# ivanalberico/End-To-End-Self-Supervised-SLAM

Hardware: AMD Instinct MI355X
Metric: online refinement steps/sec @640x480, seq_len=60 (higher is better)
Workload: dtype f32

## Files before the change

### end-to-end-self-supervised-slam_amd/csrc/conv.hip

```cpp
#include <cassert>
#include <type_traits>

#include "e2e_common.h"

typedef float f4v __attribute__((ext_vector_type(4)));
typedef float f16v __attribute__((ext_vector_type(16)));

#define CBK 16

enum { ACT_NONE = 0, ACT_RELU = 1, ACT_ELU = 2, ACT_DISP = 3 };

struct ConvArgs {
    const float* src0;
    const float* src1;
    const float* w;
    const float* scale;
    const float* shift;
    const float* res;
    float* out;
    int B, Hs, Ws;
    int Cin, C1, up;
    int Hd, Wd;
    int Ncols, ldw;
    int KH, KW, stride, pad, pad_mode;
// ... 764 lines not shown
#pragma unroll
            for (int kk = 0; kk < CB / 2; ++kk) {
                av[kk] = As[buf][kk * 2 + khalf][arow_l];
                bv[kk] = Bs[buf][kk * 2 + khalf][wn * 32 + (lane & 31)];
            }
#pragma unroll
            for (int kk = 0; kk < CB / 2; ++kk) acc = __builtin_amdgcn_mfma_f32_32x32x2f32(av[kk], bv[kk], acc, 0, 0, 0);
            __builtin_amdgcn_sched_group_barrier(0x100, CB / 2, 0);
            __builtin_amdgcn_sched_group_barrier(0x008, CB / 2, 0);
            __builtin_amdgcn_sched_barrier(0);
            store_chunk(buf ^ 1, buf ^ 1);
            __syncthreads();
        };
        {
            int c = cb;
            for (; c + 1 < ce; c += 2) {
                chunk_step(c, std::integral_constant<int, 0>{});
                chunk_step(c + 1, std::integral_constant<int, 1>{});
            }
            if (c < ce) chunk_step(c, std::integral_constant<int, 0>{});
        }
        const unsigned sl_off = (unsigned)((wave * 4 * 64 + lane) * 16);
        if (cb != 0) {
            const __amdgpu_buffer_rsrc_t rsl = __builtin_amdgcn_make_buffer_rsrc((void*)(s.slabs + (int64_t)g * (BM * BN)), 0, BM * BN * 4, 0x00020000);
            float v[16];
#pragma unroll
            for (int r = 0; r < 16; ++r) {
                v[r] = acc[r];
                asm volatile("" : "+v"(v[r]));
            }
#pragma unroll
            for (int q = 0; q < 4; ++q) {
                const f4v t = {v[4 * q], v[4 * q + 1], v[4 * q + 2], v[4 * q + 3]};
                __builtin_amdgcn_raw_buffer_store_b128(__builtin_bit_cast(__attribute__((__vector_size__(4 * sizeof(unsigned)))) unsigned, t), rsl, sl_off + q * 64 * 16, 0, SK_SC1);
            }
            asm volatile("s_waitcnt vmcnt(0)" ::: "memory");
            __syncthreads();
            if (tid == 0) __hip_atomic_store(&s.flags[g], 1u, __ATOMIC_RELAXED, __HIP_MEMORY_SCOPE_AGENT);
        } else {
            if (ce != s.C) {
                const int64_t tile_end = (int64_t)(tile + 1) * s.C;
                int h_last = g;
                for (int h = g + 1; h < s.G && s.I * h / s.G < tile_end; ++h) h_last = h;
                if (tid == 0) {
                    for (int h = g + 1; h <= h_last; ++h) {
                        unsigned spins = 0;
                        while (__hip_atomic_load(&s.flags[h], __ATOMIC_RELAXED, __HIP_MEMORY_SCOPE_AGENT) == 0u) {
                            __builtin_amdgcn_s_sleep(2);
                            if (++spins > (1u << 24)) { __hip_atomic_store(&s.flags[SK_ERR_INDEX], 1u, __ATOMIC_RELAXED, __HIP_MEMORY_SCOPE_AGENT); break; }
                        }
                    }
                    __builtin_amdgcn_fence(__ATOMIC_ACQUIRE, "agent");
                }
                asm volatile("s_waitcnt vmcnt(0)" ::: "memory");
                __syncthreads();
                for (int h = g + 1; h <= h_last; ++h) {
                    const __amdgpu_buffer_rsrc_t rsl = __builtin_amdgcn_make_buffer_rsrc((void*)(s.slabs + (int64_t)h * (BM * BN)), 0, BM * BN * 4, 0x00020000);
                    f4v t[4];
#pragma unroll
                    for (int q = 0; q < 4; ++q) t[q] = __builtin_bit_cast(f4v, __builtin_amdgcn_raw_buffer_load_b128(rsl, sl_off + q * 64 * 16, 0, SK_SC1));
#pragma unroll
                    for (int q = 0; q < 4; ++q)
#pragma unroll
                        for (int e = 0; e < 4; ++e) acc[4 * q + e] += t[q][e];
                }
                if (tid == 0)
                    for (int h = g + 1; h <= h_last; ++h) __hip_atomic_store(&s.flags[h], 0u, __ATOMIC_RELAXED, __HIP_MEMORY_SCOPE_AGENT);
            }
            const EpiRsrc er = make_epi_rsrc<TRANSPOSED>(a);
            epilogue_block<TRANSPOSED>(a, er, acc, c0 + wn * 32 + (lane & 31), n0 + wm * 32 + 4 * khalf, Ntot);
        }
        it += ce - cb;
    }
}

struct ThinArgs {
    const float* src;
    const float* w;
    const float* bias;
    float* out;
    int B, Hsrc, Wsrc, Hd, Wd, ldw, act, org, flip;
};

template <int CIN, int UP, bool REFLECT, int TH>
__global__ __launch_bounds__(256) void k_conv3x3_thin(ThinArgs a) {
    constexpr int TW = 64, PH = TH + 2, PW = TW + 2, PWS = 72, PLANE = PH * PWS, KQ = CIN / 4;
    static_assert(PLANE % 32 == 16, "the two channel planes a half-wave reads must sit 16 banks apart");
    __shared__ float patch[CIN * PLANE];
    const int tid = threadIdx.x, lane = tid & 63, wave = tid >> 6, l16 = lane & 15, kq = lane >> 4;
    const int x0 = blockIdx.x * TW, y0 = blockIdx.y * TH, b = blockIdx.z;
    const int HD = a.Hsrc * UP, WD = a.Wsrc * UP;
    float wreg[9][KQ];
#pragma unroll
    for (int t = 0; t < 9; ++t)
#pragma unroll
        for (int j = 0; j < KQ; ++j) wreg[t][j] = a.w[(int64_t)((a.flip ? 8 - t : t) * CIN + 4 * j + kq) * a.ldw + l16];
    const float* sb = a.src + (int64_t)b * a.Hsrc * a.Wsrc * CIN;
    for (int idx = tid; idx < PH * PW * KQ; idx += 256) {
        const int q = (UP == 2) ? idx / (PH * PW) : idx % KQ, pix = (UP == 2) ? idx % (PH * PW) : idx / KQ;
        const int py = pix / PW, px = pix - py * PW;
        int Y = y0 - a.org + py, X = x0 - a.org + px;
        bool ok = true;
        if (REFLECT) {
            Y = min(max(reflect1(Y, HD), 0), HD - 1);
            X = min(max(reflect1(X, WD), 0), WD - 1);
        } else {
            ok = Y >= 0 && Y < HD && X >= 0 && X < WD;
        }
        f4v v = {0.f, 0.f, 0.f, 0.f};
        if (ok) v = *(const f4v*)(sb + ((int64_t)(Y / UP) * a.Wsrc + (X / UP)) * CIN + q * 4);
#pragma unroll
        for (int e = 0; e < 4; ++e) patch[(q * 4 + e) * PLANE + py * PWS + px] = v[e];
    }
    __syncthreads();
    const float bv = a.bias ? a.bias[l16] : 0.f;
    float* ob = a.out + (int64_t)b * a.Hd * a.Wd * 16;
#pragma unroll 1
    for (int g2 = 0; g2 < TH; g2 += 2) {
        const int g0 = wave * TH + g2, g1 = g0 + 1;
        const int r0 = g0 >> 2, c0 = (g0 & 3) * 16, r1 = g1 >> 2, c1 = (g1 & 3) * 16;
        f4v acc0 = {0.f, 0.f, 0.f, 0.f}, acc1 = {0.f, 0.f, 0.f, 0.f};
        const float* p0 = patch + kq * PLANE + r0 * PWS + c0 + l16;
        const float* p1 = patch + kq * PLANE + r1 * PWS + c1 + l16;
#pragma unroll
        for (int t = 0; t < 9; ++t) {
            const int off = (t / 3) * PWS + (t % 3);
#pragma unroll
            for (int j = 0; j < KQ; ++j) {
                acc0 = __builtin_amdgcn_mfma_f32_16x16x4f32(p0[4 * j * PLANE + off], wreg[t][j], acc0, 0, 0, 0);
                acc1 = __builtin_amdgcn_mfma_f32_16x16x4f32(p1[4 * j * PLANE + off], wreg[t][j], acc1, 0, 0, 0);
            }
        }
#pragma unroll
        for (int h = 0; h < 2; ++h) {
            const f4v acc = h ? acc1 : acc0;
            const int y = y0 + (h ? r1 : r0), xb = x0 + (h ? c1 : c0) + 4 * kq;
            if (y >= a.Hd) continue;
#pragma unroll
            for (int i = 0; i < 4; ++i)
                if (xb + i < a.Wd) ob[((int64_t)y * a.Wd + xb + i) * 16 + l16] = apply_act(acc[i] + bv, a.act);
        }
    }
}

struct StemArgs {
    const float* src;
    const float* w;
    const float* scale;
    const float* shift;
    float* out;
    int B, Hs, Ws, Hd, Wd, ldw, act;
    float in_sub, in_mul;
};

__global__ __launch_bounds__(256) void k_conv7x7_stem(StemArgs a) {
    constexpr int TH = 4, TW = 32, PH = 2 * TH + 6, PW = 2 * TW + 5, ROW = 208, NJ = 37;
    __shared__ float patch[PH * ROW];
    const int tid = threadIdx.x, lane = tid & 63, wave = tid >> 6, l16 = lane & 15, kq = lane >> 4;
    const int x0 = blockIdx.x * TW, y0 = blockIdx.y * TH, b = blockIdx.z;
    const int co = 16 * wave + l16;
    float wreg[NJ];
    int offk[NJ];
#pragma unroll
    for (int j = 0; j < NJ; ++j) {
        const int k = 4 * j + kq;
        wreg[j] = k < 147 ? a.w[(int64_t)k * a.ldw + co] : 0.f;
        offk[j] = k + (k / 21) * (ROW - 21);
    }
    const float* sb = a.src + (int64_t)b * a.Hs * a.Ws * 3;
    for (int idx = tid; idx < PH * ROW; idx += 256) {
        const int py = idx / ROW, e = idx - py * ROW;
        const int Y = 2 * y0 - 3 + py, X = 2 * x0 - 3 + e / 3;
        const bool ok = e < 3 * PW && Y >= 0 && Y < a.Hs && X >= 0 && X < a.Ws;
        patch[idx] = ok ? (sb[((int64_t)Y * a.Ws + X) * 3 + (e - (e / 3) * 3)] - a.in_sub) * a.in_mul : 0.f;
    }
    __syncthreads();
    const float sc = a.scale ? a.scale[co] : 1.f, sh = a.shift ? a.shift[co] : 0.f;
    float* ob = a.out + (int64_t)b * a.Hd * a.Wd * 64;
#pragma unroll 1
    for (int g = 0; g < 2 * TH; g += 2) {
        const int r = g >> 1;
        const float* p0 = patch + 2 * r * ROW + 6 * l16;
        const float* p1 = p0 + 6 * 16;
        f4v acc0 = {0.f, 0.f, 0.f, 0.f}, acc1 = {0.f, 0.f, 0.f, 0.f};
#pragma unroll
        for (int j = 0; j < NJ; ++j) {
            acc0 = __builtin_amdgcn_mfma_f32_16x16x4f32(p0[offk[j]], wreg[j], acc0, 0, 0, 0);
            acc1 = __builtin_amdgcn_mfma_f32_16x16x4f32(p1[offk[j]], wreg[j], acc1, 0, 0, 0);
        }
        const int y = y0 + r;
        if (y >= a.Hd) continue;
#pragma unroll
        for (int h = 0; h < 2; ++h) {
            const f4v acc = h ? acc1 : acc0;
            const int xb = x0 + 16 * h + 4 * kq;
#pragma unroll
            for (int i = 0; i < 4; ++i)
                if (xb + i < a.Wd) ob[((int64_t)y * a.Wd + xb + i) * 64 + co] = apply_act(fmaf(acc[i], sc, sh), a.act);
        }
    }
}

__global__ __launch_bounds__(256) void k_conv_splitk_epilogue(const float* __restrict__ slab, int S, int64_t total, int Ncols,
                                                              const float* __restrict__ scale, const float* __restrict__ shift,
                                                              const float* res, float* out, int act, const float* __restrict__ xin, int dact,
                                                              const float* __restrict__ pre) {
    for (int64_t i = (int64_t)blockIdx.x * 256 + threadIdx.x; i < total; i += (int64_t)gridDim.x * 256) {
        float v = 0.f;
        for (int z = 0; z < S; ++z) v += slab[(int64_t)z * total + i];
        const int col = (int)(i % Ncols);
        v = fmaf(v, scale ? scale[col] : 1.f, shift ? shift[col] : 0.f);
        if (pre) v += pre[i];
        if (dact) v *= act_deriv(xin[i], dact);
        if (res) v += res[i];
        out[i] = apply_act(v, act);
    }
}

__global__ __launch_bounds__(256) void k_conv_splitk_epilogue_cls(const float* __restrict__ slab, int64_t cls_rows, int B, int Hd, int Wd, int Ncols,
                                                                  int KH, int KW, int off, const float* res, float* out, const float* __restrict__ xin,
                                                                  int dact, const float* __restrict__ pre) {
    const unsigned colq = (unsigned)Ncols >> 2, totalq = (unsigned)B * Hd * Wd * colq;
    for (unsigned q = blockIdx.x * 256u + threadIdx.x; q < totalq; q += gridDim.x * 256u) {
        unsigned t = q;
        const unsigned cq = t % colq; t /= colq;
        const unsigned x = t % Wd; t /= Wd;
        const unsigned y = t % Hd;
        const unsigned b = t / Hd;
        const int py = y & 1, px = x & 1;
        const int kh0 = (py + off) & 1, kw0 = (px + off) & 1;
        const int ntap = ((KH - kh0 + 1) / 2) * ((KW - kw0 + 1) / 2);
        const int Hc = (Hd - py + 1) / 2, Wc = (Wd - px + 1) / 2;
        const int64_t row = ((int64_t)b * Hc + (y >> 1)) * Wc + (x >> 1);
        f4v v = {0.f, 0.f, 0.f, 0.f};
        for (int z = 0; z < ntap; ++z) v += *(const f4v*)(slab + (((int64_t)z * 4 + (py * 2 + px)) * cls_rows + row) * Ncols + cq * 4);
        if (pre) v += ((const f4v*)pre)[q];
        if (dact) {
            const f4v xv = ((const f4v*)xin)[q];
#pragma unroll
            for (int k = 0; k < 4; ++k) v[k] *= act_deriv(xv[k], dact);
        }
        if (res) v += ((const f4v*)res)[q];
        ((f4v*)out)[q] = v;
    }
}

__global__ __launch_bounds__(256) void k_conv_splitk_epilogue4(const float* __restrict__ slab, int S, unsigned totalq, int Ncols,
                                                               const float* __restrict__ scale, const float* __restrict__ shift,
                                                               const float* res, float* out, int act, const float* __restrict__ xin, int dact,
                                                               const float* __restrict__ pre) {
    const unsigned colq = (unsigned)Ncols >> 2;
    for (unsigned q = blockIdx.x * 256u + threadIdx.x; q < totalq; q += gridDim.x * 256u) {
        f4v v = {0.f, 0.f, 0.f, 0.f};
        for (int z = 0; z < S; ++z) v += ((const f4v*)slab)[(int64_t)z * totalq + q];
        const int col = (int)(q % colq) * 4;
        const f4v sc = scale ? *(const f4v*)(scale + col) : (f4v){1.f, 1.f, 1.f, 1.f};
        const f4v sh = shift ? *(const f4v*)(shift + col) : (f4v){0.f, 0.f, 0.f, 0.f};
#pragma unroll
        for (int k = 0; k < 4; ++k) v[k] = fmaf(v[k], sc[k], sh[k]);
        if (pre) v += ((const f4v*)pre)[q];
        if (dact) {
            const f4v xv = ((const f4v*)xin)[q];
#pragma unroll
            for (int k = 0; k < 4; ++k) v[k] *= act_deriv(xv[k], dact);
        }
        if (res) v += ((const f4v*)res)[q];
#pragma unroll
        for (int k = 0; k < 4; ++k) v[k] = apply_act(v[k], act);
        ((f4v*)out)[q] = v;
    }
}

struct WgradArgs {
    const float* dz;
    const float* src0;
    const float* src1;
    float* slabs;
    int B, Hs, Ws, Cin, C1, up;
    int Ho, Wo, Cout;
    int KH, KW, stride, pad, pad_mode;
    int Ngemm;
// ... 1655 lines not shown
        if (workspace && cls_wgs < 500 && a.KH == 3 && a.KW == 3 && a.Cin % cb == 0 && a.Ncols % 4 == 0 && total < (1ll << 31) && !a.scale && !a.shift &&
            a.act == ACT_NONE) {
            a.ksplit = CLS_TAP_SLICES; a.cps = a.Cin / cb; a.cls_rows = Nc;
            p.g = dim3((unsigned)(4 * ((Nc + c.bm - 1) / c.bm)), (unsigned)((a.Ncols + c.bn - 1) / c.bn), (unsigned)CLS_TAP_SLICES);
            p.tail = GT_CLS;
            return p;
        }
        p.g = dim3((unsigned)(4 * ((Nc + c.bm - 1) / c.bm)), (unsigned)((a.Ncols + c.bn - 1) / c.bn));
        return p;
    }
    const GemmCfg c = choose_cfg(Ntot, a.Ncols, K, cb, workspace != nullptr, force);
    p.c = c;
    if (c.S < 0 && workspace && vec == 4 && K % cb == 0 && a.Cin % cb == 0) {
        p.kind = GK_STREAMK;
        p.G = -c.S;
        return p;
    }
    if (c.S > 1) {
        const int nchunks = (K + cb - 1) / cb;
        a.cps = (nchunks + c.S - 1) / c.S;
        const int Sz = (nchunks + a.cps - 1) / a.cps;
        a.ksplit = Sz;
        if (Sz > 1) {
            p.g = dim3((unsigned)((Ntot + c.bm - 1) / c.bm), (unsigned)((a.Ncols + c.bn - 1) / c.bn), (unsigned)Sz);
            const int64_t total = Ntot * a.Ncols;
            p.tail = (a.Ncols % 4 == 0 && total < (1ll << 31)) ? GT_SPLITK4 : GT_SPLITK;
            return p;
        }
        a.ksplit = 1; a.cps = 0;
    }
    p.g = dim3((unsigned)((Ntot + c.bm - 1) / c.bm), (unsigned)((a.Ncols + c.bn - 1) / c.bn));
    return p;
}

template <bool TR>
static void launch_gemm_main(ConvArgs& a, const GemmLaunch& p, float* workspace_all, hipStream_t st) {
    if (p.kind == GK_SCALAR) hipLaunchKernelGGL((k_conv_gemm<4, 1, 1, 2, 1, TR, 16>), p.g, dim3(256), 0, st, a);
    else if (p.kind == GK_STREAMK) launch_streamk<TR>(a, p.cb, p.G, workspace_all, st);
    else launch_tile<TR>(a, p.cb, p.c, p.g, st);
}

static void launch_gemm_tail(const ConvArgs& a, const GemmLaunch& p, hipStream_t st) {
    const int64_t total = (int64_t)a.B * a.Hd * a.Wd * a.Ncols;
    if (p.tail == GT_CLS)
        hipLaunchKernelGGL(k_conv_splitk_epilogue_cls, dim3(egrid(total / 4)), dim3(256), 0, st, a.slab, a.cls_rows, a.B, a.Hd, a.Wd, a.Ncols, a.KH, a.KW, a.off,
                           a.res, a.out, a.xin, a.dact, a.pre);
    else if (p.tail == GT_SPLITK4)
        hipLaunchKernelGGL(k_conv_splitk_epilogue4, dim3(egrid(total / 4)), dim3(256), 0, st, a.slab, a.ksplit, (unsigned)(total / 4), a.Ncols, a.scale, a.shift,
                           a.res, a.out, a.act, a.xin, a.dact, a.pre);
    else if (p.tail == GT_SPLITK)
        hipLaunchKernelGGL(k_conv_splitk_epilogue, dim3(egrid(total)), dim3(256), 0, st, a.slab, a.ksplit, total, a.Ncols, a.scale, a.shift, a.res, a.out, a.act,
                           a.xin, a.dact, a.pre);
}

template <bool TR>
static void launch_gemm(ConvArgs a, int vec, float* workspace_all, GemmCfg force, hipStream_t st) {
    const GemmLaunch p = plan_gemm<TR>(a, vec, workspace_all, force);
    launch_gemm_main<TR>(a, p, workspace_all, st);
    launch_gemm_tail(a, p, st);
}

extern "C" {

int e2e_conv_weight_layouts(const float* w, int Cout, int Cin, int KH, int KW, float* w_fwd, int ld_fwd, float* w_bwd,
                            int ld_bwd, void* stream) {
    E2E_REQUIRE(w && Cout > 0 && Cin > 0 && KH > 0 && KW > 0 && (w_fwd || w_bwd), E2E_ERR_ARG, "e2e_conv_weight_layouts: bad argument");
    E2E_REQUIRE((!w_fwd || (ld_fwd >= Cout && ld_fwd % 4 == 0)) && (!w_bwd || (ld_bwd >= Cin && ld_bwd % 4 == 0)), E2E_ERR_ARG,
                "e2e_conv_weight_layouts: leading dimensions must cover the columns and be multiples of 4");
    hipLaunchKernelGGL(k_weight_layouts, dim3(egrid((int64_t)Cout * Cin * KH * KW)), dim3(256), 0, (hipStream_t)stream, w, Cout, Cin, KH,
                       KW, w_fwd, ld_fwd, w_bwd, ld_bwd);
    E2E_LAUNCH_CHECK("e2e_conv_weight_layouts");
    return E2E_OK;
}

static int device_cus() {
    static const int cus = [] {
        int dev = 0, n = 0;
        if (hipGetDevice(&dev) != hipSuccess || hipDeviceGetAttribute(&n, hipDeviceAttributeMultiprocessorCount, dev) != hipSuccess || n <= 0) n = 256;
        return n;
    }();
    return cus;
}

int e2e_conv_weight_layouts_batched(const long long* desc, int nlayers, void* stream) {
    E2E_REQUIRE(desc && nlayers > 0, E2E_ERR_ARG, "e2e_conv_weight_layouts_batched: bad argument");
    const int grid = device_cus() * 8;
    for (int l0 = 0; l0 < nlayers; l0 += WL_MAXL)
        hipLaunchKernelGGL(k_weight_layouts_batched, dim3(grid), dim3(256), 0, (hipStream_t)stream, desc + (int64_t)l0 * 10, nlayers - l0 < WL_MAXL ? nlayers - l0 : WL_MAXL);
    E2E_LAUNCH_CHECK("e2e_conv_weight_layouts_batched");
    return E2E_OK;
}

int64_t e2e_conv2d_splitk_workspace_floats(int64_t rows, int cols, int K) {
    if (K % 16 != 0) return 0;
    int smax = 1;
    bool sk = false;
    for (int cb = 16; cb <= 32; cb += 16) {
        const GemmCfg c = choose_cfg(rows, cols, K, cb, true);
        if (c.S > smax) smax = c.S;
        if (c.S < 0) sk = true;
    }
    int64_t n = smax > 1 ? (int64_t)smax * rows * cols : 0;
    if (sk && n < (int64_t)SK_MAX_G * 64 * 64) n = (int64_t)SK_MAX_G * 64 * 64;
    return n ? n + SK_FLAG_FLOATS : 0;
}

int64_t e2e_conv2d_bwd_data_workspace_floats(int B, int Hd, int Wd, int cols, int K, int stride) {
    const int64_t plain = e2e_conv2d_splitk_workspace_floats((int64_t)B * Hd * Wd, cols, K);
    if (stride != 2) return plain;
    const int64_t cls = SK_FLAG_FLOATS + cls_slab_floats(B, Hd, Wd, cols);
    return cls > plain ? cls : plain;
}

int64_t e2e_conv_tuned_workspace_floats(int64_t rows, int cols) {
    int64_t n = (int64_t)16 * rows * cols;
    if (n < (int64_t)SK_MAX_G * 64 * 64) n = (int64_t)SK_MAX_G * 64 * 64;
    return n + SK_FLAG_FLOATS;
}
int e2e_conv_workspace_flag_floats(void) { return SK_FLAG_FLOATS; }
int e2e_conv_streamk_error_index(void) { return SK_ERR_INDEX; }

int e2e_conv_gemm_choice(int64_t rows, int cols, int K, int chunk_depth, int allow_split, int* out3) {
    E2E_REQUIRE(out3 && rows > 0 && cols > 0 && K > 0 && (chunk_depth == 16 || chunk_depth == 32), E2E_ERR_ARG, "e2e_conv_gemm_choice: bad argument");
    const GemmCfg c = choose_cfg(rows, cols, K, chunk_depth, allow_split != 0);
    out3[0] = c.bm; out3[1] = c.bn; out3[2] = c.S;
    return E2E_OK;
}

struct ConvGeom { int B, Hs, Ws, Cin, Cout, Ho, Wo, KH, KW, stride, pad, pad_mode, C1, up; float in_sub, in_mul; };
#define GEOM_LAYER(g) ConvGeom g{}; g.B = B; g.Hs = Hs; g.Ws = Ws; g.Cin = Cin; g.Cout = Cout; g.KH = KH; g.KW = KW; g.stride = stride; g.pad = pad; g.pad_mode = pad_mode
#define GEOM_SOURCES(g) g.C1 = C1; g.up = up; g.in_sub = in_sub; g.in_mul = in_mul
#define GEOM_OUTPUT(g) g.Ho = Ho; g.Wo = Wo
#define GEOM_BWD_DATA(g) GEOM_LAYER(g); GEOM_OUTPUT(g)
#define GEOM_BWD_WEIGHT(g) GEOM_LAYER(g); GEOM_OUTPUT(g); GEOM_SOURCES(g)
#define GEOM_WGRAD_QUERY(g) ConvGeom g{}; g.B = B; g.Ho = Ho; g.Wo = Wo; g.Cin = Cin; g.Cout = Cout; g.KH = KH; g.KW = KW
struct FwdOps { const float *src0, *src1, *w_fwd; int ld_fwd; const float *scale, *shift, *residual; float* out; int act; };
struct BwdDataOps { const float* dz; const float* w_bwd; int ld_bwd; float* dxp; int accumulate; const float* x_in; int in_act; const float* pre_add; };
struct WgradIn { const float *dz, *src0, *src1; float* workspace; };

static int fwd_setup(const FwdOps& f, const ConvGeom& g, ConvArgs& a_out, int& vec_out, const char* who) {
    const int B = g.B, Hs = g.Hs, Ws = g.Ws, Cin = g.Cin, Cout = g.Cout, KH = g.KH, KW = g.KW, stride = g.stride, pad = g.pad, pad_mode = g.pad_mode;
    const int C1 = g.C1, up = g.up, ld_fwd = f.ld_fwd;
    E2E_REQUIRE(f.src0 && f.w_fwd && f.out && B > 0 && Hs > 0 && Ws > 0 && Cin > 0 && Cout > 0 && KH > 0 && KW > 0, E2E_ERR_ARG, "%s: bad argument", who);
    E2E_REQUIRE(up == 1 || up == 2, E2E_ERR_ARG, "%s: upsample factor must be 1 or 2", who);
    E2E_REQUIRE(C1 > 0 && C1 <= Cin && (C1 == Cin || f.src1), E2E_ERR_ARG, "%s: bad channel split", who);
    E2E_REQUIRE(pad_mode == 0 || (pad_mode == 1 && pad == 1 && Hs >= 2 && Ws >= 2), E2E_ERR_ARG, "%s: reflection padding needs pad == 1", who);
    E2E_REQUIRE(stride == 1 || stride == 2, E2E_ERR_ARG, "%s: stride must be 1 or 2", who);
    E2E_REQUIRE(Hs % up == 0 && Ws % up == 0 && ld_fwd % 4 == 0 && ld_fwd >= Cout, E2E_ERR_ARG, "%s: bad sizes", who);
    E2E_REQUIRE(pad >= 0 && Hs + 2 * pad >= KH && Ws + 2 * pad >= KW, E2E_ERR_ARG, "%s: the kernel must fit the padded input (pad >= 0)", who);
    const int vec = (Cin % 16 == 0 && (C1 == Cin || C1 % 16 == 0)) ? 4 : 1;
    E2E_REQUIRE(vec == 4 || (C1 == Cin && up == 1), E2E_ERR_ARG, "%s: the scalar path (Cin %% 16 != 0) takes a single full-resolution source", who);
    E2E_REQUIRE((int64_t)B * Hs * Ws * Cin * 4 < (1ll << 30) && (int64_t)KH * KW * Cin * ld_fwd * 4 < (1ll << 31), E2E_ERR_ARG,
                "%s: activations must stay below 1 GB, weights below 2 GB (32-bit buffer offsets with out-of-range markers)", who);
    E2E_REQUIRE(vec != 4 || (KH <= 3 && KW <= 3), E2E_ERR_ARG, "%s: the channel-quad loader takes kernels up to 3 x 3", who);
    ConvArgs a{};
    a.src0 = f.src0; a.src1 = f.src1; a.w = f.w_fwd; a.scale = f.scale; a.shift = f.shift; a.res = f.residual; a.out = f.out;
    a.B = B; a.Hs = Hs; a.Ws = Ws; a.Cin = Cin; a.C1 = C1; a.up = up;
    a.Hd = (Hs + 2 * pad - KH) / stride + 1; a.Wd = (Ws + 2 * pad - KW) / stride + 1;
    a.Ncols = Cout; a.ldw = ld_fwd; a.KH = KH; a.KW = KW; a.stride = stride; a.pad = pad; a.pad_mode = pad_mode; a.off = 0; a.act = f.act;
    a.in_sub = g.in_sub; a.in_mul = g.in_mul;
    a_out = a; vec_out = vec;
    return E2E_OK;
}

static int conv_fwd_impl(const FwdOps& f, const ConvGeom& g, float* workspace, GemmCfg force, void* stream) {
    const int B = g.B, Hs = g.Hs, Ws = g.Ws, Cin = g.Cin, Cout = g.Cout, KH = g.KH, KW = g.KW, stride = g.stride, pad = g.pad, pad_mode = g.pad_mode;
    const int C1 = g.C1, up = g.up, ld_fwd = f.ld_fwd;
    ConvArgs a;
    int vec;
    const int rc = fwd_setup(f, g, a, vec, "e2e_conv2d_fwd");
    if (rc != E2E_OK) return rc;
    if (!force.bm && KH == 7 && KW == 7 && stride == 2 && pad == 3 && pad_mode == 0 && Cin == 3 && Cout == 64 && C1 == Cin && up == 1 && !f.residual && ld_fwd >= 64) {
        StemArgs t{f.src0, f.w_fwd, f.scale, f.shift, f.out, B, Hs, Ws, a.Hd, a.Wd, ld_fwd, f.act, g.in_sub, g.in_mul};
        hipLaunchKernelGGL(k_conv7x7_stem, dim3((a.Wd + 31) / 32, (a.Hd + 3) / 4, B), dim3(256), 0, (hipStream_t)stream, t);
    }
    else if (!force.bm && KH == 3 && KW == 3 && stride == 1 && pad == 1 && pad_mode == 1 && Cout == 16 && C1 == Cin && !f.scale && !f.residual && ld_fwd >= 16 &&
        ((Cin == 16 && up == 2) || (Cin == 32 && up == 1))) {
        ThinArgs t{f.src0, f.w_fwd, f.shift, f.out, B, Hs / up, Ws / up, Hs, Ws, ld_fwd, f.act, 1, 0};
        if (Cin == 16) hipLaunchKernelGGL((k_conv3x3_thin<16, 2, true, 8>), dim3((Ws + 63) / 64, (Hs + 7) / 8, B), dim3(256), 0, (hipStream_t)stream, t);
        else hipLaunchKernelGGL((k_conv3x3_thin<32, 1, true, 4>), dim3((Ws + 63) / 64, (Hs + 3) / 4, B), dim3(256), 0, (hipStream_t)stream, t);
    } else
        launch_gemm<false>(a, vec, workspace, force, (hipStream_t)stream);
    E2E_LAUNCH_CHECK("e2e_conv2d_fwd");
    return E2E_OK;
}

int e2e_conv2d_fwd(const float* src0, const float* src1, int C1, int up, const float* w_fwd, int ld_fwd, const float* scale,
                   const float* shift, const float* residual, float* out, int B, int Hs, int Ws, int Cin, int Cout, int KH,
                   int KW, int stride, int pad, int pad_mode, int act, float in_sub, float in_mul, float* workspace, void* stream) {
    GEOM_LAYER(g); GEOM_SOURCES(g);
    return conv_fwd_impl(FwdOps{src0, src1, w_fwd, ld_fwd, scale, shift, residual, out, act}, g, workspace, GemmCfg{0, 0, 0}, stream);
}

static bool tuning_ok(int tile_m, int tile_n, int ksplit) {
    if (tile_m == 0) return true;
    if (ksplit < 0) return tile_m == 64 && tile_n == 64 && -ksplit <= SK_MAX_G;
    return tile_max_cb(tile_m, tile_n) != 0 && ksplit >= 1 && ksplit <= 16;
}

int e2e_conv2d_fwd_tuned(const float* src0, const float* src1, int C1, int up, const float* w_fwd, int ld_fwd, const float* scale,
                         const float* shift, const float* residual, float* out, int B, int Hs, int Ws, int Cin, int Cout, int KH,
                         int KW, int stride, int pad, int pad_mode, int act, float in_sub, float in_mul, float* workspace, int tile_m, int tile_n,
                         int ksplit, void* stream) {
    E2E_REQUIRE(tuning_ok(tile_m, tile_n, ksplit), E2E_ERR_ARG, "e2e_conv2d_fwd_tuned: unsupported decomposition %d x %d / %d", tile_m, tile_n, ksplit);
    GEOM_LAYER(g); GEOM_SOURCES(g);
    return conv_fwd_impl(FwdOps{src0, src1, w_fwd, ld_fwd, scale, shift, residual, out, act}, g, workspace, GemmCfg{tile_m, tile_n, ksplit}, stream);
}

struct EntryOps {
    const float* x;
    const float *w1_fwd; int ld1; const float *scale1, *shift1; float* out1; int act1; float* workspace1;
    const float* wd_fwd; int ldd; const float *gamma, *beta, *mean, *var; float eps; float *bn_scale, *bn_shift, *bn_rstd, *z, *y;
};
struct EntryPlan { ConvArgs a1, ad; int vec1, vecd; GemmLaunch p1, pd; ConvGeom g1, gd; bool paired; };

static int fwd_entry_plan(const EntryOps& q, const ConvGeom& g, EntryPlan& P, const char* who) {
    E2E_REQUIRE(q.gamma && q.beta && q.mean && q.var && q.bn_scale && q.bn_shift && q.bn_rstd && q.z && q.y, E2E_ERR_ARG, "%s: bad argument", who);
    E2E_REQUIRE(g.pad_mode == 0 && g.C1 == g.Cin && g.up == 1, E2E_ERR_ARG, "%s: a stage entry reads one zero-padded full-resolution source", who);
    P.g1 = g;
    P.gd = g; P.gd.KH = P.gd.KW = 1; P.gd.pad = 0;
    int rc = fwd_setup(FwdOps{q.x, nullptr, q.w1_fwd, q.ld1, q.scale1, q.shift1, nullptr, q.out1, q.act1}, P.g1, P.a1, P.vec1, who);
    if (rc != E2E_OK) return rc;
    rc = fwd_setup(FwdOps{q.x, nullptr, q.wd_fwd, q.ldd, nullptr, nullptr, nullptr, q.z, ACT_NONE}, P.gd, P.ad, P.vecd, who);
    if (rc != E2E_OK) return rc;
    E2E_REQUIRE(P.a1.Hd == P.ad.Hd && P.a1.Wd == P.ad.Wd, E2E_ERR_ARG, "%s: the two branches must produce the same output grid", who);
    P.paired = false;
    if (P.vec1 != 4 || P.vecd != 4 || g.Cout < 128) return E2E_OK;
    P.p1 = plan_gemm<false>(P.a1, 4, q.workspace1, GemmCfg{0, 0, 0});
    P.pd = plan_gemm<false>(P.ad, 4, nullptr, GemmCfg{0, 0, 0});
    auto t14 = [](const GemmLaunch& p) { return p.kind == GK_TILE && p.cb == 32 && p.c.bm == 32 && p.c.bn == 128; };
    P.paired = t14(P.p1) && t14(P.pd) && P.pd.tail == GT_NONE && P.ad.ksplit == 1 && P.pd.g.z == 1;
    return E2E_OK;
}

int e2e_conv2d_fwd_entry_pair(const float* x, const float* w1_fwd, int ld1, const float* scale1, const float* shift1, float* out1, int act1,
                              float* workspace1, const float* wd_fwd, int ldd, const float* gamma, const float* beta, const float* running_mean,
                              const float* running_var, float eps, float* bn_scale, float* bn_shift, float* bn_rstd, float* z, float* y, int B, int Hs,
                              int Ws, int Cin, int Cout, int KH, int KW, int stride, int pad, void* stream) {
    const int pad_mode = 0, C1 = Cin, up = 1;
    const float in_sub = 0.f, in_mul = 1.f;
    GEOM_LAYER(g); GEOM_SOURCES(g);
    const EntryOps q{x, w1_fwd, ld1, scale1, shift1, out1, act1, workspace1, wd_fwd, ldd, gamma, beta, running_mean, running_var, eps, bn_scale, bn_shift, bn_rstd, z, y};
    EntryPlan P;
    int rc = fwd_entry_plan(q, g, P, "e2e_conv2d_fwd_entry_pair");
    if (rc != E2E_OK) return rc;
    const hipStream_t st = (hipStream_t)stream;
    if (!P.paired) {
        rc = conv_fwd_impl(FwdOps{x, nullptr, w1_fwd, ld1, scale1, shift1, nullptr, out1, act1}, P.g1, workspace1, GemmCfg{0, 0, 0}, stream);
        if (rc != E2E_OK) return rc;
        rc = conv_fwd_impl(FwdOps{x, nullptr, wd_fwd, ldd, nullptr, nullptr, nullptr, z, ACT_NONE}, P.gd, nullptr, GemmCfg{0, 0, 0}, stream);
        if (rc != E2E_OK) return rc;
        rc = e2e_bn_fold(gamma, beta, running_mean, running_var, eps, bn_scale, bn_shift, bn_rstd, Cout, stream);
        if (rc != E2E_OK) return rc;
        return e2e_affine_fwd(z, bn_scale, bn_shift, nullptr, 0, y, (int64_t)B * P.ad.Hd * P.ad.Wd * Cout, Cout, stream);
    }
    FwdPairGrid pg;
    pg.agx = P.p1.g.x; pg.agy = P.p1.g.y; pg.agz = P.p1.g.z;
    pg.bgx = P.pd.g.x; pg.bgy = P.pd.g.y;
    pg.first = (pg.agx * pg.agy * pg.agz + 7u) / 8u * 8u;
    const BnFoldArgs bn{gamma, beta, running_mean, running_var, eps, bn_scale, bn_shift, bn_rstd, y};
    hipLaunchKernelGGL(k_conv_fwd_pair, dim3(pg.first + pg.bgx * pg.bgy), dim3(256), 0, st, P.a1, P.ad, bn, pg);
    launch_gemm_tail(P.a1, P.p1, st);
    E2E_LAUNCH_CHECK("e2e_conv2d_fwd_entry_pair");
    return E2E_OK;
}

int e2e_conv2d_fwd_entry_pair_is_one_launch(int ld1, int ldd, int has_workspace1, int B, int Hs, int Ws, int Cin, int Cout, int KH, int KW, int stride, int pad) {
    static float nowhere[4];
    float* const p = nowhere;
    const int pad_mode = 0, C1 = Cin, up = 1;
    const float in_sub = 0.f, in_mul = 1.f;
    GEOM_LAYER(g); GEOM_SOURCES(g);
    const EntryOps q{p, p, ld1, p, p, p, ACT_RELU, has_workspace1 ? p : nullptr, p, ldd, p, p, p, p, 0.f, p, p, p, p, p};
    EntryPlan P;
    if (fwd_entry_plan(q, g, P, "e2e_conv2d_fwd_entry_pair_is_one_launch") != E2E_OK) return 0;
    return P.paired ? 1 : 0;
}

static int bwd_data_setup(const BwdDataOps& d, const ConvGeom& g, GemmCfg force, hipStream_t stream, ConvArgs& a, bool& done, bool dry = false) {
    const int B = g.B, Hs = g.Hs, Ws = g.Ws, Cin = g.Cin, Cout = g.Cout, Ho = g.Ho, Wo = g.Wo, KH = g.KH, KW = g.KW, stride = g.stride, pad = g.pad;
    const int pad_mode = g.pad_mode, ld_bwd = d.ld_bwd;
    done = false;
    E2E_REQUIRE(d.pre_add == nullptr || pad_mode == 0, E2E_ERR_ARG, "e2e_conv2d_bwd_data: the pre-activation addend takes a zero-padded layer");
    E2E_REQUIRE(d.in_act == 0 || (d.x_in && (d.in_act == ACT_RELU || d.in_act == ACT_ELU) && pad_mode == 0), E2E_ERR_ARG,
                "e2e_conv2d_bwd_data: the fused input-activation derivative takes ReLU / ELU, the activation's output and a zero-padded layer");
    E2E_REQUIRE(d.dz && d.w_bwd && d.dxp && B > 0 && Cin > 0 && Cout > 0 && Cout % 16 == 0, E2E_ERR_ARG, "e2e_conv2d_bwd_data: bad argument (Cout %% 16 == 0)");
    E2E_REQUIRE(ld_bwd % 4 == 0 && ld_bwd >= Cin && (stride == 1 || stride == 2), E2E_ERR_ARG, "e2e_conv2d_bwd_data: bad sizes");
    E2E_REQUIRE((int64_t)B * Ho * Wo * Cout * 4 < (1ll << 30) && (int64_t)KH * KW * Cout * ld_bwd * 4 < (1ll << 31) && KH <= 3 && KW <= 3, E2E_ERR_ARG,
                "e2e_conv2d_bwd_data: gradients must stay below 1 GB, weights below 2 GB (32-bit buffer offsets), kernels up to 3 x 3");
    if (!force.bm && KH == 3 && KW == 3 && stride == 1 && pad == 1 && pad_mode == 1 && Cin == 16 && Cout == 16 && !d.accumulate && !d.in_act && !d.pre_add && ld_bwd >= 16) {
        ThinArgs t{d.dz, d.w_bwd, nullptr, d.dxp, B, Ho, Wo, Hs + 2, Ws + 2, ld_bwd, ACT_NONE, 2, 1};
        if (!dry) hipLaunchKernelGGL((k_conv3x3_thin<16, 1, false, 8>), dim3((Ws + 2 + 63) / 64, (Hs + 2 + 7) / 8, B), dim3(256), 0, stream, t);
        done = true;
        return E2E_OK;
    }
    a = ConvArgs{};
    a.src0 = d.dz; a.src1 = nullptr; a.w = d.w_bwd; a.out = d.dxp;
    a.B = B; a.Hs = Ho; a.Ws = Wo; a.Cin = Cout; a.C1 = Cout; a.up = 1;
    const int pp = pad_mode == 1 ? pad : 0;
    a.Hd = Hs + 2 * pp; a.Wd = Ws + 2 * pp; a.off = pad_mode == 1 ? 0 : pad;
    a.Ncols = Cin; a.ldw = ld_bwd; a.KH = KH; a.KW = KW; a.stride = stride; a.pad = pad; a.pad_mode = 0; a.act = ACT_NONE;
    a.cls = (stride == 2 && cls_rows(B, a.Hd, a.Wd) < (1 << 24)) ? 1 : 0;
    if (a.cls && (KH < 2 || KW < 2) && !d.accumulate && !dry)
        (void)hipMemsetAsync(d.dxp, 0, (size_t)B * a.Hd * a.Wd * Cin * sizeof(float), stream);
    if (d.accumulate) a.res = d.dxp;
    a.xin = d.in_act ? d.x_in : nullptr; a.dact = d.in_act; a.pre = d.pre_add;
    return E2E_OK;
}

static int bwd_data_impl(const BwdDataOps& d, const ConvGeom& g, float* workspace, void* stream, GemmCfg force = GemmCfg{0, 0, 0}) {
    ConvArgs a;
    bool done;
    const int rc = bwd_data_setup(d, g, force, (hipStream_t)stream, a, done);
    if (rc != E2E_OK) return rc;
    if (!done) launch_gemm<true>(a, 4, workspace, force, (hipStream_t)stream);
    E2E_LAUNCH_CHECK("e2e_conv2d_bwd_data");
    return E2E_OK;
}

int e2e_conv2d_bwd_data(const float* dz, const float* w_bwd, int ld_bwd, float* dxp, int B, int Hs, int Ws, int Cin, int Cout,
                        int Ho, int Wo, int KH, int KW, int stride, int pad, int pad_mode, float* workspace, void* stream) {
    GEOM_BWD_DATA(g);
    return bwd_data_impl(BwdDataOps{dz, w_bwd, ld_bwd, dxp, 0, nullptr, 0, nullptr}, g, workspace, stream);
}

int e2e_conv2d_bwd_data_acc(const float* dz, const float* w_bwd, int ld_bwd, float* dxp, int B, int Hs, int Ws, int Cin, int Cout,
                            int Ho, int Wo, int KH, int KW, int stride, int pad, int pad_mode, int accumulate, float* workspace,
                            void* stream) {
    GEOM_BWD_DATA(g);
    return bwd_data_impl(BwdDataOps{dz, w_bwd, ld_bwd, dxp, accumulate, nullptr, 0, nullptr}, g, workspace, stream);
}

int e2e_conv2d_bwd_data_fused(const float* da, const float* w_bwd, int ld_bwd, float* dxp, int B, int Hs, int Ws, int Cin, int Cout,
                              int Ho, int Wo, int KH, int KW, int stride, int pad, int pad_mode, int accumulate, const float* x_in,
                              int in_act, const float* pre_add, float* workspace, void* stream) {
    GEOM_BWD_DATA(g);
    return bwd_data_impl(BwdDataOps{da, w_bwd, ld_bwd, dxp, accumulate, x_in, in_act, pre_add}, g, workspace, stream);
}

int e2e_conv2d_bwd_data_fused_tuned(const float* da, const float* w_bwd, int ld_bwd, float* dxp, int B, int Hs, int Ws, int Cin, int Cout,
                                    int Ho, int Wo, int KH, int KW, int stride, int pad, int pad_mode, int accumulate, const float* x_in,
                                    int in_act, const float* pre_add, float* workspace, int tile_m, int tile_n, int ksplit, void* stream) {
    E2E_REQUIRE(tuning_ok(tile_m, tile_n, ksplit), E2E_ERR_ARG, "e2e_conv2d_bwd_data_fused_tuned: unsupported decomposition %d x %d / %d", tile_m, tile_n, ksplit);
    GEOM_BWD_DATA(g);
    return bwd_data_impl(BwdDataOps{da, w_bwd, ld_bwd, dxp, accumulate, x_in, in_act, pre_add}, g, workspace, stream, GemmCfg{tile_m, tile_n, ksplit});
}

struct GatherAdjoint { const float* dxp; int B, Hs, Ws, Cin, C1, up, padded; float *d0, *d1; int acc0, acc1; const float* x0; int act0; const float* x1; int act1; };
static void launch_gather_adjoint(const GatherAdjoint& q, hipStream_t st) {
    const int64_t n = (int64_t)q.B * (q.Hs / q.up) * (q.Ws / q.up) * q.C1 + (int64_t)q.B * q.Hs * q.Ws * (q.Cin - q.C1);
    if (q.Cin % 4 == 0 && q.C1 % 4 == 0 && n < (1ll << 31))
        hipLaunchKernelGGL(k_gather_adjoint4, dim3(egrid(n / 4)), dim3(256), 0, st, q.dxp, q.B, q.Hs, q.Ws, q.Cin, q.C1, q.up, q.padded ? 1 : 0, q.d0, q.d1, q.acc0, q.acc1,
                           q.x0, q.act0, q.x1, q.act1);
    else
        hipLaunchKernelGGL(k_gather_adjoint, dim3(egrid(n)), dim3(256), 0, st, q.dxp, q.B, q.Hs, q.Ws, q.Cin, q.C1, q.up, q.padded ? 1 : 0, q.d0, q.d1, q.acc0, q.acc1,
                           q.x0, q.act0, q.x1, q.act1);
}

int e2e_conv2d_gather_adjoint(const float* dxp, int B, int Hs, int Ws, int Cin, int C1, int up, int padded, float* d_src0,
                              float* d_src1, int accumulate0, int accumulate1, void* stream) {
    E2E_REQUIRE(dxp && d_src0 && B > 0 && Cin > 0 && C1 > 0 && C1 <= Cin && (C1 == Cin || d_src1) && (up == 1 || up == 2), E2E_ERR_ARG,
                "e2e_conv2d_gather_adjoint: bad argument");
    launch_gather_adjoint(GatherAdjoint{dxp, B, Hs, Ws, Cin, C1, up, padded, d_src0, d_src1, accumulate0, accumulate1, nullptr, 0, nullptr, 0}, (hipStream_t)stream);
    E2E_LAUNCH_CHECK("e2e_conv2d_gather_adjoint");
    return E2E_OK;
}

int e2e_conv2d_gather_adjoint_act(const float* dxp, int B, int Hs, int Ws, int Cin, int C1, int up, int padded, float* d_src0, float* d_src1,
                                  int accumulate0, int accumulate1, const float* src0, int act0, const float* src1, int act1, void* stream) {
    E2E_REQUIRE(dxp && d_src0 && B > 0 && Cin > 0 && C1 > 0 && C1 <= Cin && (C1 == Cin || d_src1) && (up == 1 || up == 2), E2E_ERR_ARG,
                "e2e_conv2d_gather_adjoint_act: bad argument");
    E2E_REQUIRE((act0 == 0 || src0) && (act1 == 0 || src1) && act0 >= 0 && act0 <= 2 && act1 >= 0 && act1 <= 2, E2E_ERR_ARG,
                "e2e_conv2d_gather_adjoint_act: an activation derivative needs the activation's output");
    launch_gather_adjoint(GatherAdjoint{dxp, B, Hs, Ws, Cin, C1, up, padded, d_src0, d_src1, accumulate0, accumulate1, src0, act0, src1, act1}, (hipStream_t)stream);
    E2E_LAUNCH_CHECK("e2e_conv2d_gather_adjoint_act");
// ... 408 lines not shown
```

Before: 225.6.

## Add persistent software-pipelined patch loading to thin 3x3 and 7x7 stem convs

Adds persistent-grid variants of the thin 3x3 conv kernels and the 7x7 stem conv. Each workgroup loops over tiles and prefetches the next tile's input patch into registers through buffer loads while the MFMA sweep runs on the current patch in shared memory. The aim is to hide global-load latency and cut the cost of one-shot workgroup launches. It also loads the low-resolution source once for the upsampled case and writes each value to four patch positions. The cost is extra register pressure from the prefetch registers and an extra barrier per tile. Both paths are on by default, and environment switches can turn them off.

```diff
diff --git a/end-to-end-self-supervised-slam_amd/csrc/conv.hip b/end-to-end-self-supervised-slam_amd/csrc/conv.hip
--- a/end-to-end-self-supervised-slam_amd/csrc/conv.hip
+++ b/end-to-end-self-supervised-slam_amd/csrc/conv.hip
@@ -870,12 +870,15 @@
     int B, Hsrc, Wsrc, Hd, Wd, ldw, act, org, flip;
 };
 
+template <int CIN, int TH>
+__device__ __forceinline__ void thin_sweep(const ThinArgs& a, const float* patch, const float (&wreg)[9][CIN / 4], float bv, int x0, int y0, int b);
+
 template <int CIN, int UP, bool REFLECT, int TH>
 __global__ __launch_bounds__(256) void k_conv3x3_thin(ThinArgs a) {
     constexpr int TW = 64, PH = TH + 2, PW = TW + 2, PWS = 72, PLANE = PH * PWS, KQ = CIN / 4;
     static_assert(PLANE % 32 == 16, "the two channel planes a half-wave reads must sit 16 banks apart");
     __shared__ float patch[CIN * PLANE];
-    const int tid = threadIdx.x, lane = tid & 63, wave = tid >> 6, l16 = lane & 15, kq = lane >> 4;
+    const int tid = threadIdx.x, lane = tid & 63, l16 = lane & 15, kq = lane >> 4;
     const int x0 = blockIdx.x * TW, y0 = blockIdx.y * TH, b = blockIdx.z;
     const int HD = a.Hsrc * UP, WD = a.Wsrc * UP;
     float wreg[9][KQ];
@@ -902,6 +905,13 @@
     }
     __syncthreads();
     const float bv = a.bias ? a.bias[l16] : 0.f;
+    thin_sweep<CIN, TH>(a, patch, wreg, bv, x0, y0, b);
+}
+
+template <int CIN, int TH>
+__device__ __forceinline__ void thin_sweep(const ThinArgs& a, const float* patch, const float (&wreg)[9][CIN / 4], float bv, int x0, int y0, int b) {
+    constexpr int PWS = 72, PLANE = (TH + 2) * PWS, KQ = CIN / 4;
+    const int lane = threadIdx.x & 63, wave = threadIdx.x >> 6, l16 = lane & 15, kq = lane >> 4;
     float* ob = a.out + (int64_t)b * a.Hd * a.Wd * 16;
 #pragma unroll 1
     for (int g2 = 0; g2 < TH; g2 += 2) {
@@ -927,6 +937,106 @@
 #pragma unroll
             for (int i = 0; i < 4; ++i)
                 if (xb + i < a.Wd) ob[((int64_t)y * a.Wd + xb + i) * 16 + l16] = apply_act(acc[i] + bv, a.act);
+        }
+    }
+}
+
+template <int CIN, int UP, bool REFLECT, int TH>
+__global__ __launch_bounds__(256) void k_conv3x3_thin_pipe(ThinArgs a, int ntx, int nty, int ntiles) {
+    constexpr int TW = 64, PH = TH + 2, PW = TW + 2, PWS = 72, PLANE = PH * PWS, KQ = CIN / 4;
+    constexpr int SR = TH / 2 + 2, SC = TW / 2 + 2;
+    constexpr int NL = UP == 2 ? (SR * SC * KQ + 255) / 256 : PH * (KQ / 4) + 1;
+    constexpr unsigned OOB = 0x80000000u;
+    static_assert(PLANE % 32 == 16, "the two channel planes a half-wave reads must sit 16 banks apart");
+    static_assert(UP == 1 || (UP == 2 && REFLECT && TH % 2 == 0), "the upsampled form is the reflection-padded forward");
+    static_assert(KQ % 4 == 0 && PH * 2 * KQ <= 256, "UP == 1 loads: a wave per channel quad, the two edge columns in one pass");
+    __shared__ float patch[CIN * PLANE];
+    const int tid = threadIdx.x, lane = tid & 63, wave = tid >> 6, l16 = lane & 15, kq = lane >> 4;
+    const int HD = a.Hsrc * UP, WD = a.Wsrc * UP;
+    float wreg[9][KQ];
+#pragma unroll
+    for (int t = 0; t < 9; ++t)
+#pragma unroll
+        for (int j = 0; j < KQ; ++j) wreg[t][j] = a.w[(int64_t)((a.flip ? 8 - t : t) * CIN + 4 * j + kq) * a.ldw + l16];
+    const float bv = a.bias ? a.bias[l16] : 0.f;
+    const __amdgpu_buffer_rsrc_t rs = __builtin_amdgcn_make_buffer_rsrc((void*)a.src, 0, a.B * a.Hsrc * a.Wsrc * CIN * 4, 0x00020000);
+    const int epy = min(tid / (2 * KQ), PH - 1), epx = TW + ((tid / KQ) & 1), eq = tid % KQ;
+    f4v preg[NL];
+    auto fetch = [&](int off) { return __builtin_bit_cast(f4v, __builtin_amdgcn_raw_buffer_load_b128(rs, (unsigned)off, 0, 0)); };
+    auto load_patch = [&](int tile) {
+        const int tx = tile % ntx, ty = (tile / ntx) % nty, b = tile / (ntx * nty);
+        const int x0 = tx * TW, y0 = ty * TH, pb = b * a.Hsrc * a.Wsrc;
+        if constexpr (UP == 2) {
+#pragma unroll
+            for (int i = 0; i < NL; ++i) {
+                const int idx = tid + 256 * i, q = idx / (SR * SC), pix = idx - q * (SR * SC), sr = pix / SC, sc = pix - sr * SC;
+                const int Y = min(max(y0 / 2 - 1 + sr, 0), a.Hsrc - 1), X = min(max(x0 / 2 - 1 + sc, 0), a.Wsrc - 1);
+                preg[i] = fetch(idx < SR * SC * KQ ? ((pb + Y * a.Wsrc + X) * CIN + q * 4) * 4 : (int)OOB);
+            }
+        } else {
+            auto col = [&](int px) {
+                const int X = x0 - a.org + px;
+                if (REFLECT) return min(max(reflect1(X, WD), 0), WD - 1) * CIN;
+                return X >= 0 && X < WD ? X * CIN : -1;
+            };
+            auto row = [&](int py) {
+                const int Y = y0 - a.org + py;
+                if (REFLECT) return (pb + min(max(reflect1(Y, HD), 0), HD - 1) * a.Wsrc) * CIN;
+                return Y >= 0 && Y < HD ? (pb + Y * a.Wsrc) * CIN : -1;
+            };
+            const int c = col(lane), ce = col(epx), re = row(epy);
+#pragma unroll
+            for (int py = 0; py < PH; ++py) {
+                const int r = row(py);
+#pragma unroll
+                for (int p = 0; p < KQ / 4; ++p) preg[py * (KQ / 4) + p] = fetch((r | c) >= 0 ? (r + c + (4 * p + wave) * 4) * 4 : (int)OOB);
+            }
+            preg[NL - 1] = fetch((re | ce) >= 0 ? (re + ce + eq * 4) * 4 : (int)OOB);
+        }
+    };
+    auto store_patch = [&]() {
+        if constexpr (UP == 2) {
+#pragma unroll
+            for (int i = 0; i < NL; ++i) {
+                const int idx = tid + 256 * i, q = idx / (SR * SC), pix = idx - q * (SR * SC), sr = pix / SC, sc = pix - sr * SC;
+                if (idx >= SR * SC * KQ) continue;
+#pragma unroll
+                for (int dy = 0; dy < 2; ++dy)
+#pragma unroll
+                    for (int dx = 0; dx < 2; ++dx) {
+                        const int py = 2 * sr - 1 + dy, px = 2 * sc - 1 + dx;
+                        if (py < 0 || py >= PH || px < 0 || px >= PW) continue;
+#pragma unroll
+                        for (int e = 0; e < 4; ++e) patch[(q * 4 + e) * PLANE + py * PWS + px] = preg[i][e];
+                    }
+            }
+        } else {
+#pragma unroll
+            for (int py = 0; py < PH; ++py)
+#pragma unroll
+                for (int p = 0; p < KQ / 4; ++p)
+#pragma unroll
+                    for (int e = 0; e < 4; ++e) patch[((4 * p + wave) * 4 + e) * PLANE + py * PWS + lane] = preg[py * (KQ / 4) + p][e];
+            if (tid < PH * 2 * KQ)
+#pragma unroll
+                for (int e = 0; e < 4; ++e) patch[(eq * 4 + e) * PLANE + epy * PWS + epx] = preg[NL - 1][e];
+        }
+    };
+    const int nwg = gridDim.x;
+    int tile = blockIdx.x;
+    if (tile < ntiles) {
+        load_patch(tile);
+        store_patch();
+    }
+    __syncthreads();
+    for (; tile < ntiles; tile += nwg) {
+        const bool more = tile + nwg < ntiles;
+        if (more) load_patch(tile + nwg);
+        thin_sweep<CIN, TH>(a, patch, wreg, bv, (tile % ntx) * TW, ((tile / ntx) % nty) * TH, tile / (ntx * nty));
+        __syncthreads();
+        if (more) {
+            store_patch();
+            __syncthreads();
         }
     }
 }
@@ -941,6 +1051,9 @@
     float in_sub, in_mul;
 };
 
+__device__ __forceinline__ void stem_sweep(const StemArgs& a, const float* patch, const float (&wreg)[37], const int (&offk)[37], float sc, float sh,
+                                           int x0, int y0, int b);
+
 __global__ __launch_bounds__(256) void k_conv7x7_stem(StemArgs a) {
     constexpr int TH = 4, TW = 32, PH = 2 * TH + 6, PW = 2 * TW + 5, ROW = 208, NJ = 37;
     __shared__ float patch[PH * ROW];
@@ -964,6 +1077,13 @@
     }
     __syncthreads();
     const float sc = a.scale ? a.scale[co] : 1.f, sh = a.shift ? a.shift[co] : 0.f;
+    stem_sweep(a, patch, wreg, offk, sc, sh, x0, y0, b);
+}
+
+__device__ __forceinline__ void stem_sweep(const StemArgs& a, const float* patch, const float (&wreg)[37], const int (&offk)[37], float sc, float sh,
+                                           int x0, int y0, int b) {
+    constexpr int TH = 4, ROW = 208, NJ = 37;
+    const int lane = threadIdx.x & 63, wave = threadIdx.x >> 6, l16 = lane & 15, kq = lane >> 4, co = 16 * wave + l16;
     float* ob = a.out + (int64_t)b * a.Hd * a.Wd * 64;
 #pragma unroll 1
     for (int g = 0; g < 2 * TH; g += 2) {
@@ -985,6 +1105,64 @@
 #pragma unroll
             for (int i = 0; i < 4; ++i)
                 if (xb + i < a.Wd) ob[((int64_t)y * a.Wd + xb + i) * 64 + co] = apply_act(fmaf(acc[i], sc, sh), a.act);
+        }
+    }
+}
+
+__global__ __launch_bounds__(256) __attribute__((amdgpu_waves_per_eu(5))) void k_conv7x7_stem_pipe(StemArgs a, int ntx, int nty, int ntiles) {
+    constexpr int TH = 4, TW = 32, PH = 2 * TH + 6, PW = 2 * TW + 5, ROW = 208, NJ = 37;
+    constexpr unsigned OOB = 0x80000000u;
+    __shared__ float patch[PH * ROW];
+    const int tid = threadIdx.x, lane = tid & 63, wave = tid >> 6, l16 = lane & 15, kq = lane >> 4;
+    const int co = 16 * wave + l16;
+    float wreg[NJ];
+    int offk[NJ];
+#pragma unroll
+    for (int j = 0; j < NJ; ++j) {
+        const int k = 4 * j + kq;
+        wreg[j] = k < 147 ? a.w[(int64_t)k * a.ldw + co] : 0.f;
+        offk[j] = k + (k / 21) * (ROW - 21);
+    }
+    const float sc = a.scale ? a.scale[co] : 1.f, sh = a.shift ? a.shift[co] : 0.f;
+    const __amdgpu_buffer_rsrc_t rs = __builtin_amdgcn_make_buffer_rsrc((void*)a.src, 0, a.B * a.Hs * a.Ws * 3 * 4, 0x00020000);
+    float preg[PH];
+    bool colok = false;
+    auto load_patch = [&](int tile) {
+        const int x0 = (tile % ntx) * TW, y0 = ((tile / ntx) % nty) * TH, pb = (tile / (ntx * nty)) * a.Hs;
+        const int X = 2 * x0 - 3 + tid / 3;
+        colok = tid < 3 * PW && X >= 0 && X < a.Ws;
+        const int c = 6 * x0 - 9 + tid;
+#pragma unroll
+        for (int py = 0; py < PH; ++py) {
+            const int Y = 2 * y0 - 3 + py;
+            const bool ok = colok && Y >= 0 && Y < a.Hs;
+            preg[py] = __builtin_bit_cast(float, __builtin_amdgcn_raw_buffer_load_b32(rs, ok ? (unsigned)(((pb + Y) * a.Ws * 3 + c) * 4) : OOB, 0, 0));
+        }
+    };
+    auto store_patch = [&](int tile) {
+        const int y0 = ((tile / ntx) % nty) * TH;
+        if (tid < ROW)
+#pragma unroll
+            for (int py = 0; py < PH; ++py) {
+                const int Y = 2 * y0 - 3 + py;
+                patch[py * ROW + tid] = colok && Y >= 0 && Y < a.Hs ? (preg[py] - a.in_sub) * a.in_mul : 0.f;
+            }
+    };
+    const int nwg = gridDim.x;
+    int tile = blockIdx.x;
+    if (tile < ntiles) {
+        load_patch(tile);
+        store_patch(tile);
+    }
+    __syncthreads();
+    for (; tile < ntiles; tile += nwg) {
+        const bool more = tile + nwg < ntiles;
+        if (more) load_patch(tile + nwg);
+        stem_sweep(a, patch, wreg, offk, sc, sh, (tile % ntx) * TW, ((tile / ntx) % nty) * TH, tile / (ntx * nty));
+        __syncthreads();
+        if (more) {
+            store_patch(tile + nwg);
+            __syncthreads();
         }
     }
 }
@@ -2806,6 +2984,25 @@
     return cus;
 }
 
+static bool patch_pipeline_on(const char* part_switch) {
+    const char* all = getenv("E2E_PATCH_PIPELINE");
+    const char* one = getenv(part_switch);
+    return !(all && all[0] == '0') && !(one && one[0] == '0');
+}
+
+static int resident_workgroups(const void* kernel) {
+    int n = 0;
+    if (hipOccupancyMaxActiveBlocksPerMultiprocessor(&n, kernel, 256, 0) != hipSuccess || n < 1) n = 1;
+    return n;
+}
+
+static int patch_deal(int tiles, int resident) {
+    const char* ev = getenv("E2E_PATCH_WGS");
+    const int forced = ev ? atoi(ev) : 0;
+    if (forced > 0) return std::min(forced, 1 << 20);
+    return std::min(tiles, resident * device_cus());
+}
+
 int e2e_conv_weight_layouts_batched(const long long* desc, int nlayers, void* stream) {
     E2E_REQUIRE(desc && nlayers > 0, E2E_ERR_ARG, "e2e_conv_weight_layouts_batched: bad argument");
     const int grid = device_cus() * 8;
@@ -2896,13 +3093,28 @@
     if (rc != E2E_OK) return rc;
     if (!force.bm && KH == 7 && KW == 7 && stride == 2 && pad == 3 && pad_mode == 0 && Cin == 3 && Cout == 64 && C1 == Cin && up == 1 && !f.residual && ld_fwd >= 64) {
         StemArgs t{f.src0, f.w_fwd, f.scale, f.shift, f.out, B, Hs, Ws, a.Hd, a.Wd, ld_fwd, f.act, g.in_sub, g.in_mul};
-        hipLaunchKernelGGL(k_conv7x7_stem, dim3((a.Wd + 31) / 32, (a.Hd + 3) / 4, B), dim3(256), 0, (hipStream_t)stream, t);
+        const int ntx = (a.Wd + 31) / 32, nty = (a.Hd + 3) / 4;
+        if (!patch_pipeline_on("E2E_PATCH_PIPELINE_STEM")) {
+            hipLaunchKernelGGL(k_conv7x7_stem, dim3(ntx, nty, B), dim3(256), 0, (hipStream_t)stream, t);
+        } else {
+            static const int resident = std::min(4, resident_workgroups((const void*)k_conv7x7_stem_pipe));
+            hipLaunchKernelGGL(k_conv7x7_stem_pipe, dim3(patch_deal(ntx * nty * B, resident)), dim3(256), 0, (hipStream_t)stream, t, ntx, nty, ntx * nty * B);
+        }
     }
     else if (!force.bm && KH == 3 && KW == 3 && stride == 1 && pad == 1 && pad_mode == 1 && Cout == 16 && C1 == Cin && !f.scale && !f.residual && ld_fwd >= 16 &&
         ((Cin == 16 && up == 2) || (Cin == 32 && up == 1))) {
         ThinArgs t{f.src0, f.w_fwd, f.shift, f.out, B, Hs / up, Ws / up, Hs, Ws, ld_fwd, f.act, 1, 0};
-        if (Cin == 16) hipLaunchKernelGGL((k_conv3x3_thin<16, 2, true, 8>), dim3((Ws + 63) / 64, (Hs + 7) / 8, B), dim3(256), 0, (hipStream_t)stream, t);
-        else hipLaunchKernelGGL((k_conv3x3_thin<32, 1, true, 4>), dim3((Ws + 63) / 64, (Hs + 3) / 4, B), dim3(256), 0, (hipStream_t)stream, t);
+        const int ntx = (Ws + 63) / 64, nty = (Hs + (Cin == 16 ? 7 : 3)) / (Cin == 16 ? 8 : 4);
+        if (!patch_pipeline_on("E2E_PATCH_PIPELINE_THIN")) {
+            if (Cin == 16) hipLaunchKernelGGL((k_conv3x3_thin<16, 2, true, 8>), dim3(ntx, nty, B), dim3(256), 0, (hipStream_t)stream, t);
+            else hipLaunchKernelGGL((k_conv3x3_thin<32, 1, true, 4>), dim3(ntx, nty, B), dim3(256), 0, (hipStream_t)stream, t);
+        } else if (Cin == 16) {
+            static const int resident = resident_workgroups((const void*)k_conv3x3_thin_pipe<16, 2, true, 8>);
+            hipLaunchKernelGGL((k_conv3x3_thin_pipe<16, 2, true, 8>), dim3(patch_deal(ntx * nty * B, resident)), dim3(256), 0, (hipStream_t)stream, t, ntx, nty, ntx * nty * B);
+        } else {
+            static const int resident = resident_workgroups((const void*)k_conv3x3_thin_pipe<32, 1, true, 4>);
+            hipLaunchKernelGGL((k_conv3x3_thin_pipe<32, 1, true, 4>), dim3(patch_deal(ntx * nty * B, resident)), dim3(256), 0, (hipStream_t)stream, t, ntx, nty, ntx * nty * B);
+        }
     } else
         launch_gemm<false>(a, vec, workspace, force, (hipStream_t)stream);
     E2E_LAUNCH_CHECK("e2e_conv2d_fwd");
@@ -3014,7 +3226,14 @@
                 "e2e_conv2d_bwd_data: gradients must stay below 1 GB, weights below 2 GB (32-bit buffer offsets), kernels up to 3 x 3");
     if (!force.bm && KH == 3 && KW == 3 && stride == 1 && pad == 1 && pad_mode == 1 && Cin == 16 && Cout == 16 && !d.accumulate && !d.in_act && !d.pre_add && ld_bwd >= 16) {
         ThinArgs t{d.dz, d.w_bwd, nullptr, d.dxp, B, Ho, Wo, Hs + 2, Ws + 2, ld_bwd, ACT_NONE, 2, 1};
-        if (!dry) hipLaunchKernelGGL((k_conv3x3_thin<16, 1, false, 8>), dim3((Ws + 2 + 63) / 64, (Hs + 2 + 7) / 8, B), dim3(256), 0, stream, t);
+        const int ntx = (Ws + 2 + 63) / 64, nty = (Hs + 2 + 7) / 8;
+        if (dry) {
+        } else if (!patch_pipeline_on("E2E_PATCH_PIPELINE_THIN")) {
+            hipLaunchKernelGGL((k_conv3x3_thin<16, 1, false, 8>), dim3(ntx, nty, B), dim3(256), 0, stream, t);
+        } else {
+            static const int resident = resident_workgroups((const void*)k_conv3x3_thin_pipe<16, 1, false, 8>);
+            hipLaunchKernelGGL((k_conv3x3_thin_pipe<16, 1, false, 8>), dim3(patch_deal(ntx * nty * B, resident)), dim3(256), 0, stream, t, ntx, nty, ntx * nty * B);
+        }
         done = true;
         return E2E_OK;
     }
```

New measurement: 226.5, median of 6. Within noise of the previous version (+0.4%).
